# microsoft/fadtk

Measured on NVIDIA H100. Metric: audio_seconds_embedded_per_second, higher is better.
Workload: dtype f16

## Files before the change

fadtk_b200/csrc/conv_gemm.cuh:

```cuda
#pragma once
#include "sm90.cuh"

namespace fad {

struct ConvGemmParams {
    int taps;
    int cblks;
    int box_w, box_h, box_n;
    int tiles_w, tiles_h;
    int img_groups;
    int n_tiles;
    int H, W, NB, Cout;
    int lo_adds;
    int ld_out, n_valid;
    int relu, pool;
    const float* bias;
    __half* out;
    float* out_f32;
    float* resid;
    int resid_C, resid_res, resid_shift;
};

__device__ __forceinline__ long long window_row_to_token(long long o, int res, int shift) {
    const int lg_nw = 28 - __clz(res);
    const int nw = res >> 3;
    const int in = (int)(o & 63);
    const long long wi = o >> 6;
    const int wx = (int)wi & (nw - 1);
    const int wy = (int)(wi >> lg_nw) & (nw - 1);
    const long long b = wi >> (2 * lg_nw);
    int y = wy * 8 + (in >> 3) + shift, xx = wx * 8 + (in & 7) + shift;
    if (y >= res) y -= res;
    if (xx >= res) xx -= res;
    return (b * res + y) * res + xx;
}

constexpr int kTileM = 128;
constexpr int kBlockK = 64;
constexpr int kConvGemmThreads = 512;
constexpr int kConsumers = 2;
constexpr int kConsumerRegs = 168;
constexpr int kEpiRegs = 136;
constexpr int kClusterCtas = 2;
constexpr int kChunkSteps = 8;
constexpr float kAccumShrinkPerElement = 1.06e-9f;
constexpr uint32_t kABytes = kTileM * kBlockK * 2;
constexpr uint32_t kEpiRowBytes = 128 * 4;
constexpr uint32_t kEpiBytes = 64 * kEpiRowBytes;
constexpr uint32_t kBiasBytes = 128 * 4;
static_assert(40 + kEpiRegs + kConsumers * kConsumerRegs <= 65536 / 128, "register file over-subscribed");
static_assert(kConsumerRegs > 65536 / kConvGemmThreads, "the consumers raise their register count (setmaxnreg.inc)");

template <int N_TILE, int WMODE>
__host__ __device__ constexpr uint32_t conv_gemm_stage_bytes() {
    return kABytes + (WMODE == 1 ? 2 : 1) * N_TILE * kBlockK * 2;
}

template <int N_TILE, int STAGES, int WMODE>
__host__ __device__ constexpr uint32_t conv_gemm_smem_bytes() {
    return STAGES * conv_gemm_stage_bytes<N_TILE, WMODE>() + 1024  + 256
         + kConsumers * kEpiBytes + 4 * kBiasBytes;
}

__device__ __forceinline__ uint32_t pack_half2(float a, float b) {
    __half2 h = __floats2half2_rn(a, b);
    return *reinterpret_cast<uint32_t*>(&h);
}
template <int N>
__device__ __forceinline__ void gelu_erf_n(float* x) {
    float z[N], q[N];
#pragma unroll
    for (int i = 0; i < N; ++i) { z[i] = fminf(fabsf(x[i]) * 0.70710678118654752f, 4.3f); q[i] = 1.04899843e-04f; }
    constexpr float kQ[6] = {-4.92790774e-04f, -2.22368206e-03f, 2.93586859e-02f, -1.48908889e-01f, -9.18342944e-01f,
                             -1.62791250e+00f};
#pragma unroll
    for (int t = 0; t < 6; ++t) {
#pragma unroll
        for (int i = 0; i < N; ++i) q[i] = fmaf(q[i], z[i], kQ[t]);
    }
#pragma unroll
    for (int i = 0; i < N; ++i) asm("ex2.approx.ftz.f32 %0, %1;" : "=f"(q[i]) : "f"(q[i] * z[i]));
#pragma unroll
    for (int i = 0; i < N; ++i) x[i] = 0.5f * x[i] * (1.0f + copysignf(1.0f - q[i], x[i]));
}
__device__ __forceinline__ float gelu_erf(float x) {
    gelu_erf_n<1>(&x);
    return x;
}

template <int N>
__device__ __forceinline__ void elu_ex2_n(float* x) {
    float e[N], t[N];
#pragma unroll
    for (int i = 0; i < N; ++i) asm("ex2.approx.ftz.f32 %0, %1;" : "=f"(e[i]) : "f"(fminf(x[i], 0.f) * 1.4426950408889634f));
#pragma unroll
    for (int i = 0; i < N; ++i) t[i] = x[i] * fmaf(x[i], fmaf(x[i], fmaf(x[i], 4.16666667e-2f, 1.66666667e-1f), 0.5f), 1.0f);
#pragma unroll
    for (int i = 0; i < N; ++i) x[i] = x[i] > 0.f ? x[i] : (x[i] > -0.0625f ? t[i] : e[i] - 1.0f);
}

__device__ __forceinline__ uint32_t hmax2_u32(uint32_t a, uint32_t b) {
    __half2 r = __hmax2(*reinterpret_cast<__half2*>(&a), *reinterpret_cast<__half2*>(&b));
    return *reinterpret_cast<uint32_t*>(&r);
}

template <int N_TILE, int STAGES, int WMODE>
__global__ void __launch_bounds__(kConvGemmThreads, 1)
conv_gemm_kernel(const __grid_constant__ CUtensorMap map_x,
                 const __grid_constant__ CUtensorMap map_w,
                 const ConvGemmParams p)
{
    using namespace sm90;
    static_assert(N_TILE == 128, "one m64n128 accumulator per consumer warpgroup");
    static_assert(WMODE == 0 || WMODE == 1, "WMODE 0: fp16 weights, 1: fp16 hi/lo pair");
    static_assert(kClusterCtas == 2, "the work units below are M-tile pairs");
    constexpr bool SPLIT_W = WMODE == 1;
    constexpr uint32_t kStageBytes = conv_gemm_stage_bytes<N_TILE, WMODE>();
    constexpr int kBRows = (SPLIT_W ? 2 : 1) * N_TILE;
    constexpr int kGroups = N_TILE / 32;

    extern __shared__ uint8_t smem_raw[];
    uint8_t* smem = reinterpret_cast<uint8_t*>((reinterpret_cast<uintptr_t>(smem_raw) + 1023) & ~uintptr_t(1023));
    uint64_t* bars = reinterpret_cast<uint64_t*>(smem + STAGES * kStageBytes);
    uint64_t* full = bars;
    uint64_t* empty = bars + STAGES;
    uint64_t* epi_full = bars + 2 * STAGES;
    uint64_t* epi_empty = bars + 2 * STAGES + kConsumers;
    static_assert((2 * STAGES + 2 * kConsumers) * 8 <= 256, "barriers");
    uint8_t* epi = smem + STAGES * kStageBytes + 256;

    const int warp = threadIdx.x >> 5;
    const int lane = threadIdx.x & 31;
    const int ksteps = p.taps * p.cblks;
    const int n_chunks = (ksteps + kChunkSteps - 1) / kChunkSteps;
    const int chunk_len = (ksteps + n_chunks - 1) / n_chunks;
    const int m_tiles = p.img_groups * p.tiles_h * p.tiles_w;
    const int n_clusters = (int)gridDim.x / kClusterCtas;
    const int total_units = (m_tiles + 1) / 2 * p.n_tiles;

    if (warp == 0 && lane == 0) {
        tma_prefetch_desc(&map_x);
        tma_prefetch_desc(&map_w);
    }
    if (warp == 1 && lane == 0) {
        for (int s = 0; s < STAGES; ++s) { mbar_init(&full[s], 1); mbar_init(&empty[s], kClusterCtas * kConsumers * 4); }
        for (int c = 0; c < kConsumers; ++c) { mbar_init(&epi_full[c], 128); mbar_init(&epi_empty[c], 64); }
        mbar_fence_init();
    }
    cluster_sync();

    if (warp < 4) {
        setmaxnreg_dec<40>();
        if (warp == 0 && elect_one()) {
            const int rank = (int)cluster_ctarank();
            const int cluster = (int)cluster_index();
            constexpr int kHalfRows = kBRows / kClusterCtas;
            uint8_t* const w_half = smem + kABytes + rank * kHalfRows * 128;
            int s = 0; uint32_t ph = 0;
            for (int unit = cluster; unit < total_units; unit += n_clusters) {
                const int nt = unit % p.n_tiles;
                const int m = min(2 * (unit / p.n_tiles) + rank, m_tiles - 1);
                const int w0 = (m % p.tiles_w) * p.box_w;
                const int h0 = ((m / p.tiles_w) % p.tiles_h) * p.box_h;
                const int n0 = (m / (p.tiles_w * p.tiles_h)) * p.box_n;
                for (int ks = 0; ks < ksteps; ++ks) {
                    const int tap = ks / p.cblks;
                    const int cb = ks - tap * p.cblks;
                    int dh = 0, dw = 0;
                    if (p.taps == 9) { dh = tap / 3 - 1; dw = tap % 3 - 1; }
                    mbar_wait(&empty[s], ph ^ 1);
                    uint8_t* st = smem + s * kStageBytes;
                    mbar_expect_tx(&full[s], kStageBytes);
                    tma_load_4d(st, &map_x, &full[s], cb * kBlockK, w0 + dw, h0 + dh, n0);
                    tma_load_2d_multicast(w_half + s * kStageBytes, &map_w, &full[s], ks * kBlockK,
                                          nt * kBRows + rank * kHalfRows, (1u << kClusterCtas) - 1);
                    if (++s == STAGES) { s = 0; ph ^= 1; }
                }
            }
        }
    } else if (warp < 4 + 4 * kConsumers) {
        setmaxnreg_inc<kConsumerRegs>();
        const int cluster = (int)cluster_index();
        const int c = (warp >> 2) - 1;
        const int wq = warp & 3;
        const uint32_t epi_base = smem_u32(epi) + c * kEpiBytes;
        int s = 0; uint32_t ph = 0, eph = 0;
        auto release = [&](int st_) {
            __syncwarp();
            if (lane == 0) {
#pragma unroll
                for (int cta = 0; cta < kClusterCtas; ++cta) mbar_arrive_cluster(&empty[st_], cta);
            }
        };

        for (int unit = cluster; unit < total_units; unit += n_clusters) {
            float sum[64], acc[64];
#pragma unroll
            for (int i = 0; i < 64; ++i) sum[i] = 0.f;
            for (int ks0 = 0; ks0 < ksteps; ks0 += chunk_len) {
                const int ks1 = min(ks0 + chunk_len, ksteps);
                const float unshrink = kAccumShrinkPerElement * (float)((ks1 - ks0) * kBlockK * (SPLIT_W && p.lo_adds ? 2 : 1));
                int prev_s = -1;
                for (int ks = ks0; ks < ks1; ++ks) {
                    mbar_wait(&full[s], ph);
                    const uint32_t a_addr = smem_u32(smem + s * kStageBytes);
                    const uint64_t a_desc = kmajor_sw128_desc(a_addr + c * 64 * 128);
                    const uint64_t b_desc = kmajor_sw128_desc(a_addr + kABytes);
                    wgmma_fence();
#pragma unroll
                    for (int k = 0; k < kBlockK / 16; ++k) {
                        wgmma_m64n128k16_f16<0, 0>(acc, a_desc + 2 * k, b_desc + 2 * k, (ks > ks0) || (k > 0));
                        if (SPLIT_W)
                            wgmma_m64n128k16_f16<0, 0>(acc, a_desc + 2 * k, b_desc + 2 * k + (N_TILE * 128 / 16), 1);
                    }
                    wgmma_commit();
                    wgmma_wait<1>();
                    if (prev_s >= 0) release(prev_s);
                    prev_s = s;
                    if (++s == STAGES) { s = 0; ph ^= 1; }
                }
                wgmma_wait<0>();
                fence_regs(acc);
                release(prev_s);
#pragma unroll
                for (int i = 0; i < 64; ++i) sum[i] += fmaf(acc[i], unshrink, acc[i]);
            }

            mbar_wait(&epi_empty[c], eph ^ 1);
            const int fr = wq * 16 + (lane >> 2);
            const uint32_t x = ((lane & 3) >> 1) ^ (fr & 7);
            const uint32_t row_base = epi_base + fr * kEpiRowBytes + (lane & 1) * 8;
#pragma unroll
            for (int jl = 0; jl < 4; ++jl) {
                const uint32_t a = row_base + (((2 * jl) ^ x) << 4);
#pragma unroll
                for (int jh = 0; jh < 4; ++jh) {
#pragma unroll
                    for (int i = 0; i < 2; ++i) {
                        const int j = 4 * jh + jl;
                        sts64(a + i * 8 * kEpiRowBytes + jh * 128, sum[4 * j + 2 * i], sum[4 * j + 2 * i + 1]);
                    }
                }
            }
            mbar_arrive(&epi_full[c]);
            eph ^= 1;
        }
    } else {
        if constexpr (kEpiRegs > 65536 / kConvGemmThreads) setmaxnreg_inc<kEpiRegs>();
        else setmaxnreg_dec<kEpiRegs>();
        const int rank = (int)cluster_ctarank();
        const int cluster = (int)cluster_index();
        const int e = warp - 4 - 4 * kConsumers;
        const int c = e >> 1;
        const int rr = (e & 1) * 32 + lane;
        const int r = c * 64 + rr;
        const int bw = p.box_w, bh = p.box_h;
        const int pw = r % bw;
        const int phh = (r / bw) % bh;
        const int pn = r / (bw * bh);
        const uint32_t wrows = smem_u32(epi) + c * kEpiBytes + (e & 1) * 32 * kEpiRowBytes;
        const uint32_t row_mine = wrows + lane * kEpiRowBytes;
        const uint32_t bias_s = smem_u32(epi) + kConsumers * kEpiBytes + e * kBiasBytes;
        const int sw = lane & 7;
        const int cq = lane & 7, rq = lane >> 3;
        uint32_t eph = 0;
        const bool plain = p.tiles_w == 1 && p.tiles_h == 1 && bw == 1 && bh == 1;
        const bool f32_path = p.out_f32 != nullptr || p.resid != nullptr;
        auto prefetch_resid = [&](int nt_, int m_) {
            if (p.resid == nullptr || !plain) return;
            const int n_ = m_ * kTileM + r;
            if (n_ >= p.NB) return;
            const long long tok = p.resid_res ? window_row_to_token((long long)n_, p.resid_res, p.resid_shift) : (long long)n_;
            for (int cc = nt_ * N_TILE; cc < nt_ * N_TILE + N_TILE && cc < p.resid_C; cc += 32)
                asm volatile("prefetch.global.L2 [%0];" :: "l"(p.resid + tok * p.resid_C + cc));
        };
        if (cluster < total_units) prefetch_resid(cluster % p.n_tiles, 2 * (cluster / p.n_tiles) + rank);

        for (int unit = cluster; unit < total_units; unit += n_clusters) {
            const int nt = unit % p.n_tiles;
            const int m = 2 * (unit / p.n_tiles) + rank;
            if (unit + n_clusters < total_units)
                prefetch_resid((unit + n_clusters) % p.n_tiles, 2 * ((unit + n_clusters) / p.n_tiles) + rank);
            __syncwarp();
            {
                const float4 b = __ldg(reinterpret_cast<const float4*>(p.bias + nt * N_TILE) + lane);
                sts128(bias_s + lane * 16, __float_as_uint(b.x), __float_as_uint(b.y), __float_as_uint(b.z), __float_as_uint(b.w));
            }
            __syncwarp();

            int w, h, n;
            if (plain) { w = 0; h = 0; n = m * kTileM + r; }
            else {
                w = (m % p.tiles_w) * bw + pw;
                h = ((m / p.tiles_w) % p.tiles_h) * bh + phh;
                n = (m / (p.tiles_w * p.tiles_h)) * p.box_n + pn;
            }
            const bool valid = n < p.NB;
            const int ch0 = nt * N_TILE;
            long long out_off = -1, res_off = -1;
            if (valid && !p.pool) {
                out_off = (long long)((size_t(n) * p.H + h) * p.W + w) * p.ld_out;
                if (p.resid != nullptr)
                    res_off = (p.resid_res ? window_row_to_token((long long)n, p.resid_res, p.resid_shift) : (long long)n)
                              * p.resid_C;
            }

            mbar_wait(&epi_full[c], eph);
#pragma unroll 1
            for (int g = 0; g < kGroups; ++g) {
                float f[32];
#pragma unroll
                for (int j = 0; j < 8; ++j) {
                    const uint4 u = lds128(row_mine + g * 128 + ((j ^ sw) << 4));
                    const uint4 b = lds128(bias_s + g * 128 + j * 16);
                    f[4 * j + 0] = __uint_as_float(u.x) + __uint_as_float(b.x);
                    f[4 * j + 1] = __uint_as_float(u.y) + __uint_as_float(b.y);
                    f[4 * j + 2] = __uint_as_float(u.z) + __uint_as_float(b.z);
                    f[4 * j + 3] = __uint_as_float(u.w) + __uint_as_float(b.w);
                }
                if (p.relu == 1) {
#pragma unroll
                    for (int j = 0; j < 32; ++j) f[j] = fmaxf(f[j], 0.0f);
                } else if (p.relu == 2) {
#pragma unroll
                    for (int j = 0; j < 32; j += 8) gelu_erf_n<8>(f + j);
                } else if (p.relu == 3) {
#pragma unroll
                    for (int j = 0; j < 32; j += 8) elu_ex2_n<8>(f + j);
                }

                if (!p.pool) {
                    if (f32_path) {
                        if (p.out != nullptr && out_off >= 0) {
                            uint4* dst = reinterpret_cast<uint4*>(p.out + out_off + ch0 + g * 32);
#pragma unroll
                            for (int j = 0; j < 4; ++j)
                                if (ch0 + g * 32 + 8 * j < p.n_valid)
                                    dst[j] = make_uint4(pack_half2(f[8 * j], f[8 * j + 1]), pack_half2(f[8 * j + 2], f[8 * j + 3]),
                                                        pack_half2(f[8 * j + 4], f[8 * j + 5]), pack_half2(f[8 * j + 6], f[8 * j + 7]));
                        }
#pragma unroll
                        for (int j = 0; j < 8; ++j)
                            sts128(row_mine + g * 128 + ((j ^ sw) << 4), __float_as_uint(f[4 * j]), __float_as_uint(f[4 * j + 1]),
                                   __float_as_uint(f[4 * j + 2]), __float_as_uint(f[4 * j + 3]));
                        __syncwarp();
                        const int col = ch0 + g * 32 + cq * 4;
#pragma unroll
                        for (int hf = 0; hf < 2; ++hf) {
                            float4 v[4];
#pragma unroll
                            for (int it = 0; it < 4; ++it) {
                                const int x = (hf * 4 + it) * 4 + rq;
                                const uint4 u = lds128(wrows + x * kEpiRowBytes + g * 128 + ((cq ^ (x & 7)) << 4));
                                v[it] = make_float4(__uint_as_float(u.x), __uint_as_float(u.y), __uint_as_float(u.z), __uint_as_float(u.w));
                            }
                            if (p.out_f32 != nullptr) {
#pragma unroll
                                for (int it = 0; it < 4; ++it) {
                                    const long long off = __shfl_sync(0xffffffffu, out_off, (hf * 4 + it) * 4 + rq);
                                    if (off >= 0 && col < p.n_valid) *reinterpret_cast<float4*>(p.out_f32 + off + col) = v[it];
                                }
                            }
                            if (p.resid != nullptr && ch0 + g * 32 < p.resid_C) {
                                long long offs[4];
                                float4 xv[4];
#pragma unroll
                                for (int it = 0; it < 4; ++it) {
                                    offs[it] = __shfl_sync(0xffffffffu, res_off, (hf * 4 + it) * 4 + rq);
                                    if (offs[it] >= 0) xv[it] = *reinterpret_cast<const float4*>(p.resid + offs[it] + col);
                                }
#pragma unroll
                                for (int it = 0; it < 4; ++it) {
                                    if (offs[it] >= 0) {
                                        const float4 a = v[it];
                                        xv[it].x += a.x; xv[it].y += a.y; xv[it].z += a.z; xv[it].w += a.w;
                                        *reinterpret_cast<float4*>(p.resid + offs[it] + col) = xv[it];
                                    }
                                }
                            }
                        }
                    } else if (p.out != nullptr) {
                        const int seg = (g & ~1) * 128;
#pragma unroll
                        for (int j = 0; j < 4; ++j)
                            sts128(row_mine + seg + ((((g & 1) * 4 + j) ^ sw) << 4),
                                   pack_half2(f[8 * j], f[8 * j + 1]), pack_half2(f[8 * j + 2], f[8 * j + 3]),
                                   pack_half2(f[8 * j + 4], f[8 * j + 5]), pack_half2(f[8 * j + 6], f[8 * j + 7]));
                        if (g & 1) {
                            __syncwarp();
                            const int col = ch0 + (g - 1) * 32 + cq * 8;
#pragma unroll
                            for (int it = 0; it < 8; ++it) {
                                const int x = it * 4 + rq;
                                const uint4 v = lds128(wrows + x * kEpiRowBytes + seg + ((cq ^ (x & 7)) << 4));
                                const long long off = __shfl_sync(0xffffffffu, out_off, x);
                                if (off >= 0 && col < p.n_valid) *reinterpret_cast<uint4*>(p.out + off + col) = v;
                            }
                        }
                    }
                } else {
                    uint32_t h2[16];
#pragma unroll
                    for (int j = 0; j < 16; ++j) h2[j] = pack_half2(f[2 * j], f[2 * j + 1]);
#pragma unroll
                    for (int j = 0; j < 16; ++j) {
                        uint32_t o = __shfl_xor_sync(0xffffffffu, h2[j], 1);
                        h2[j] = hmax2_u32(h2[j], o);
                        o = __shfl_xor_sync(0xffffffffu, h2[j], bw);
                        h2[j] = hmax2_u32(h2[j], o);
                    }
                    const int sub = (pw & 1) | ((phh & 1) << 1);
                    uint4 o;
                    o.x = sub == 0 ? h2[0] : sub == 1 ? h2[4] : sub == 2 ? h2[8]  : h2[12];
                    o.y = sub == 0 ? h2[1] : sub == 1 ? h2[5] : sub == 2 ? h2[9]  : h2[13];
                    o.z = sub == 0 ? h2[2] : sub == 1 ? h2[6] : sub == 2 ? h2[10] : h2[14];
                    o.w = sub == 0 ? h2[3] : sub == 1 ? h2[7] : sub == 2 ? h2[11] : h2[15];
                    if (valid) {
                        const size_t pix = (size_t(n) * (p.H >> 1) + (h >> 1)) * (p.W >> 1) + (w >> 1);
                        *reinterpret_cast<uint4*>(p.out + pix * p.Cout + ch0 + g * 32 + sub * 8) = o;
                    }
                }
            }
            mbar_arrive(&epi_empty[c]);
            eph ^= 1;
        }
    }
    cluster_sync();
}

}
```

fadtk_b200/csrc/fadtk_b200.cu:

```cuda
#include "../../include/fadtk_b200.h"

#include <cuda.h>
#include <cuda_runtime.h>
#include <cuda_fp16.h>
#include <cxxabi.h>
#include <algorithm>
#include <cmath>
#include <cstdio>
#include <cstdlib>
#include <cstring>
#include <memory>
#include <set>
#include <string>
#include <type_traits>
#include <utility>
#include <vector>

#include "conv_gemm.cuh"
#include "frontend.cuh"
#include "stats.cuh"
#include "frechet.cuh"
#include "clap.cuh"
#include "resample.cuh"
#include "whisper.cuh"
#include "encodec.cuh"
#include "wav2vec.cuh"
#include "attention_wgmma.cuh"
#include "kad.cuh"
#include "prdc.cuh"

namespace {

thread_local std::string g_err;

int fail(const std::string& m) { g_err = m; return 1; }

#define CK(call)                                                                          \
    do {                                                                                  \
        cudaError_t e_ = (call);                                                          \
        if (e_ != cudaSuccess)                                                            \
            return fail(std::string(#call) + ": " + cudaGetErrorString(e_));              \
    } while (0)

class DeviceBuffer {
public:
    DeviceBuffer() = default;
    DeviceBuffer(DeviceBuffer&& o) noexcept : p_(o.p_), bytes_(o.bytes_) { o.p_ = nullptr; o.bytes_ = 0; }
    ~DeviceBuffer() { if (p_) cudaFree(p_); }

    int grow(size_t bytes) {
        if (bytes_ >= bytes) return 0;
        if (p_) cudaFree(p_);
        p_ = nullptr; bytes_ = 0;
        CK(cudaMalloc(&p_, bytes));
        bytes_ = bytes;
        return 0;
    }
    template <typename T = void> T* get() const { return static_cast<T*>(p_); }
    size_t size() const { return bytes_; }

private:
    void* p_ = nullptr;
    size_t bytes_ = 0;
};

template <typename T>
int upload(std::vector<DeviceBuffer>& mem, T** dst, const void* src, size_t bytes) {
    DeviceBuffer b;
    if (b.grow(bytes)) return 1;
    CK(cudaMemcpy(b.get(), src, bytes, cudaMemcpyHostToDevice));
    *dst = b.get<T>();
    mem.push_back(std::move(b));
    return 0;
}
template <typename T>
int alloc(std::vector<DeviceBuffer>& mem, T** dst, size_t bytes, bool zero = false) {
    DeviceBuffer b;
    if (b.grow(bytes)) return 1;
    if (zero) CK(cudaMemset(b.get(), 0, bytes));
    *dst = b.get<T>();
    mem.push_back(std::move(b));
    return 0;
}

int check_tensors(const char* fn, const void* const* t, int n_tensors) {
    for (int i = 0; i < n_tensors; ++i)
        if (!t[i]) return fail(std::string(fn) + ": null tensor pointer");
    return 0;
}

typedef CUresult (*EncodeTiledFn)(CUtensorMap*, CUtensorMapDataType, cuuint32_t, void*,
                                  const cuuint64_t*, const cuuint64_t*, const cuuint32_t*,
                                  const cuuint32_t*, CUtensorMapInterleave, CUtensorMapSwizzle,
                                  CUtensorMapL2promotion, CUtensorMapFloatOOBfill);

EncodeTiledFn get_encode_fn() {
    static EncodeTiledFn fn = nullptr;
    if (!fn) {
        void* p = nullptr;
        cudaDriverEntryPointQueryResult q;
        if (cudaGetDriverEntryPoint("cuTensorMapEncodeTiled", &p, cudaEnableDefault, &q) == cudaSuccess &&
            q == cudaDriverEntryPointSuccess)
            fn = reinterpret_cast<EncodeTiledFn>(p);
    }
    return fn;
}

int encode_f16_map(CUtensorMap* map, const void* base, int rank, const uint64_t* dims,
                   const uint64_t* strides_bytes , const uint32_t* box) {
    EncodeTiledFn fn = get_encode_fn();
    if (!fn) return fail("cuTensorMapEncodeTiled entry point not available");
    cuuint64_t gdim[5], gstr[4];
    cuuint32_t bdim[5], estr[5];
    for (int i = 0; i < rank; ++i) { gdim[i] = dims[i]; bdim[i] = box[i]; estr[i] = 1; }
    for (int i = 0; i + 1 < rank; ++i) gstr[i] = strides_bytes[i];
    CUresult r = fn(map, CU_TENSOR_MAP_DATA_TYPE_FLOAT16, (cuuint32_t)rank, const_cast<void*>(base),
                    gdim, gstr, bdim, estr, CU_TENSOR_MAP_INTERLEAVE_NONE, CU_TENSOR_MAP_SWIZZLE_128B,
                    CU_TENSOR_MAP_L2_PROMOTION_L2_256B, CU_TENSOR_MAP_FLOAT_OOB_FILL_NONE);
    if (r != CUDA_SUCCESS) {
        char buf[256];
        snprintf(buf, sizeof buf, "cuTensorMapEncodeTiled failed (%d) rank=%d dims=%llu,%llu box=%u,%u", (int)r, rank,
                 (unsigned long long)dims[0], (unsigned long long)(rank > 1 ? dims[1] : 0), box[0], rank > 1 ? box[1] : 0);
        return fail(buf);
    }
    return 0;
}

struct LayerGeom {
    int taps, Cin, Cout, H, W, relu, pool;
    int box_w, box_h, box_n, n_tile;
    int split_w;
};

int make_geom(LayerGeom& g, int H, int W, int Cin, int Cout, int taps, int relu, int pool, int split_w) {
    g.taps = taps; g.Cin = Cin; g.Cout = Cout; g.H = H; g.W = W; g.relu = relu; g.pool = pool;
    g.split_w = split_w;
    if (Cin % 64 != 0) return fail("Cin must be a multiple of 64");
    if (taps != 1 && taps != 9) return fail("taps must be 1 or 9");
    if (H == 1 && W == 1) { g.box_w = 1; g.box_h = 1; g.box_n = 128; }
    else {
        g.box_w = W < 16 ? W : 16;
        if (g.box_w != 8 && g.box_w != 16) return fail("W must be 8 or a multiple of 16");
        if (W % g.box_w != 0) return fail("W must be a multiple of the 16-pixel box");
        int bh = 1;
        while (bh * 2 <= 128 / g.box_w && H % (bh * 2) == 0) bh *= 2;
        g.box_h = bh;
        g.box_n = 128 / (g.box_w * g.box_h);
    }
    if (pool && (g.box_h % 2 != 0 || g.box_w % 2 != 0)) return fail("pooling needs even tile boxes");
    if (Cout % 128 != 0) return fail("Cout must be a multiple of 128");
    g.n_tile = 128;
    return 0;
}

struct VggState;
struct ClapState;
struct WhisperState;
struct EncodecState;
struct W2vState;

}

struct fad_handle {
    int device = 0;
    int num_sms = 0;
    int max_examples = 0;
    long long launches = 0;
    int gemm_clusters[2] = {};

    std::vector<DeviceBuffer> mem;
    double *d_twiddle = nullptr, *d_hann = nullptr, *d_melw = nullptr;
    int *d_mel_start = nullptr, *d_mel_count = nullptr;

    DeviceBuffer ws_tiles, ws_sums, gather_buf;
    DeviceBuffer fr_buf;
    DeviceBuffer rs_bank, rs_mono;
    int rs_in = 0, rs_out = 0;
    DeviceBuffer kad_buf;
    DeviceBuffer kad_agree;
    std::set<const void*> zero_lo;

    void* nccl_comm = nullptr;

    std::unique_ptr<VggState> vgg;
    std::unique_ptr<ClapState> clap;
    std::unique_ptr<WhisperState> whisper;
    std::unique_ptr<EncodecState> encodec;
    std::unique_ptr<W2vState> w2v;
    ~fad_handle();

    bool prof_on = false;
    std::vector<cudaEvent_t> ev_pool;
    size_t ev_used = 0;
    struct Span { int cat; size_t e0, e1; };
    std::vector<Span> spans;
    double prof_ms[FAD_PROF_CATEGORIES] = {};
    long long prof_count[FAD_PROF_CATEGORIES] = {};
};

namespace {

std::string kernel_name(const void* kernel) {
    const char* mangled = nullptr;
    if (cudaFuncGetName(&mangled, kernel) != cudaSuccess || !mangled) return "kernel launch";
    int status = 0;
    char* demangled = abi::__cxa_demangle(mangled, nullptr, nullptr, &status);
    const std::string name = demangled ? demangled : mangled;
    free(demangled);
    return name;
}

template <typename... Params, typename... Args>
int launch_attrs(fad_handle* h, void (*kernel)(Params...), dim3 grid, dim3 block, size_t smem, cudaStream_t st,
                 cudaLaunchAttribute* attrs, unsigned n_attrs, Args&&... args) {
    if (grid.x == 0 || grid.y == 0 || grid.z == 0) return 0;
    cudaLaunchConfig_t cfg = {};
    cfg.gridDim = grid;
    cfg.blockDim = block;
    cfg.dynamicSmemBytes = smem;
    cfg.stream = st;
    cfg.attrs = attrs;
    cfg.numAttrs = n_attrs;
    cudaError_t e = cudaLaunchKernelEx(&cfg, kernel, std::forward<Args>(args)...);
    const cudaError_t last = cudaGetLastError();
    if (e == cudaSuccess) e = last;
    if (e != cudaSuccess) return fail(kernel_name((const void*)kernel) + ": " + cudaGetErrorString(e));
    h->launches++;
    return 0;
}
template <typename... Params, typename... Args>
int launch(fad_handle* h, void (*kernel)(Params...), dim3 grid, dim3 block, size_t smem, cudaStream_t st, Args&&... args) {
    return launch_attrs(h, kernel, grid, block, smem, st, nullptr, 0, std::forward<Args>(args)...);
}

template <int WMODE> struct Gemm {
    static constexpr int kStages = WMODE ? 3 : 4;
    static constexpr uint32_t kSmem = fad::conv_gemm_smem_bytes<128, kStages, WMODE>();
    static_assert(kSmem <= 227 * 1024, "over the per-CTA shared-memory limit");
    static constexpr auto kernel = fad::conv_gemm_kernel<128, kStages, WMODE>;
};

cudaLaunchAttribute cta_pair() {
    cudaLaunchAttribute attr = {};
    attr.id = cudaLaunchAttributeClusterDimension;
    attr.val.clusterDim.x = fad::kClusterCtas; attr.val.clusterDim.y = 1; attr.val.clusterDim.z = 1;
    return attr;
}

template <int WMODE>
int setup_gemm(fad_handle* h) {
    CK(cudaFuncSetAttribute(Gemm<WMODE>::kernel, cudaFuncAttributeMaxDynamicSharedMemorySize, (int)Gemm<WMODE>::kSmem));
    cudaLaunchAttribute attr = cta_pair();
    cudaLaunchConfig_t cfg = {};
    cfg.gridDim = dim3(fad::kClusterCtas * (unsigned)h->num_sms);
    cfg.blockDim = dim3(fad::kConvGemmThreads);
    cfg.dynamicSmemBytes = Gemm<WMODE>::kSmem;
    cfg.attrs = &attr;
    cfg.numAttrs = 1;
    CK(cudaOccupancyMaxActiveClusters(&h->gemm_clusters[WMODE], Gemm<WMODE>::kernel, &cfg));
    if (h->gemm_clusters[WMODE] <= 0) return fail("conv_gemm_kernel: no CTA pair fits on the device");
    return 0;
}

template <int WMODE>
int launch_conv_gemm(fad_handle* h, const CUtensorMap& mx, const CUtensorMap& mw, const fad::ConvGemmParams& p, cudaStream_t st) {
    const int units = (p.img_groups * p.tiles_h * p.tiles_w + 1) / 2 * p.n_tiles;
    cudaLaunchAttribute attr = cta_pair();
    return launch_attrs(h, Gemm<WMODE>::kernel, dim3(fad::kClusterCtas * (unsigned)std::min(units, h->gemm_clusters[WMODE])),
                        dim3(fad::kConvGemmThreads), Gemm<WMODE>::kSmem, st, &attr, 1, mx, mw, p);
}

int encode_layer_maps(const LayerGeom& g, const void* x, long long nb_dim, const void* w,
                      CUtensorMap* mx, CUtensorMap* mw, int a_cols = 0, long long a_row_stride = 0) {
    const uint64_t ac = a_cols > 0 ? (uint64_t)a_cols : (uint64_t)g.Cin;
    const uint64_t xd[4] = {ac, (uint64_t)g.W, (uint64_t)g.H, (uint64_t)nb_dim};
    uint64_t xs[3] = {ac * 2, (uint64_t)g.W * ac * 2, (uint64_t)g.H * g.W * ac * 2};
    if (a_row_stride > 0) xs[0] = xs[1] = xs[2] = (uint64_t)a_row_stride * 2;
    const uint32_t xb[4] = {64, (uint32_t)g.box_w, (uint32_t)g.box_h, (uint32_t)g.box_n};
    if (encode_f16_map(mx, x, 4, xd, xs, xb)) return 1;
    const uint64_t K = (uint64_t)g.taps * g.Cin;
    const uint64_t rows_mul = g.split_w ? 2 : 1;
    const uint64_t wd[2] = {K, (uint64_t)g.Cout * rows_mul};
    const uint64_t ws[1] = {K * 2};
    const uint32_t wb[2] = {64, (uint32_t)(g.n_tile * rows_mul / fad::kClusterCtas)};
    return encode_f16_map(mw, w, 2, wd, ws, wb);
}

int launch_attention_wgmma(fad_handle* h, const __half* qkv, long long n_clips, int S, int d, int heads, __half* out, cudaStream_t st) {
    if (heads * 64 != d) return fail("attention_wgmma: head dimension must be 64");
    CUtensorMap map;
    const uint64_t dims[3] = {(uint64_t)3 * d, (uint64_t)S, (uint64_t)n_clips};
    const uint64_t strides[2] = {(uint64_t)3 * d * 2, (uint64_t)S * 3 * d * 2};
    const uint32_t box[3] = {64, 128, 1};
    if (encode_f16_map(&map, qkv, 3, dims, strides, box)) return 1;
    fad::AttnParams p;
    p.S = S; p.d = d; p.heads = heads; p.out = out;
    return launch(h, fad::attention_wgmma_kernel, dim3((S + 127) / 128, heads, (unsigned)n_clips), fad::kAtThreads, fad::kAtSmem,
                  st, map, p);
}

int run_layer(fad_handle* h, const LayerGeom& g, const CUtensorMap& mx, const CUtensorMap& mw, const void* w,
              int NB, const float* bias, void* out, float* out_f32, cudaStream_t st,
              float* resid = nullptr, int resid_C = 0, int resid_res = 0, int resid_shift = 0, int n_valid = 0) {
    fad::ConvGemmParams p;
    p.taps = g.taps; p.cblks = g.Cin / 64;
    p.box_w = g.box_w; p.box_h = g.box_h; p.box_n = g.box_n;
    p.tiles_w = g.W / g.box_w; p.tiles_h = g.H / g.box_h;
    p.img_groups = (NB + g.box_n - 1) / g.box_n;
    p.n_tiles = g.Cout / g.n_tile;
    p.H = g.H; p.W = g.W; p.NB = NB; p.Cout = g.Cout;
    p.n_valid = n_valid > 0 ? n_valid : g.Cout;
    p.ld_out = p.n_valid;
    p.relu = g.relu; p.pool = g.pool;
    p.bias = bias; p.out = reinterpret_cast<__half*>(out); p.out_f32 = out_f32;
    p.resid = resid; p.resid_C = resid_C; p.resid_res = resid_res; p.resid_shift = resid_shift;
    p.lo_adds = g.split_w == 1 && h->zero_lo.count(w) == 0;
    if (g.split_w) return launch_conv_gemm<1>(h, mx, mw, p, st);
    return launch_conv_gemm<0>(h, mx, mw, p, st);
}

__global__ void wlo_absmax_kernel(const __half* __restrict__ w, long long n_tiles, long long K, unsigned int* __restrict__ out) {
    float m = 0.f;
    const long long total = n_tiles * 128 * K;
    for (long long e = blockIdx.x * (long long)blockDim.x + threadIdx.x; e < total; e += (long long)gridDim.x * blockDim.x) {
        const long long row = e / K, k = e - row * K;
        const long long t = row >> 7, j = row & 127;
        m = fmaxf(m, fabsf(__half2float(w[((t * 256 + 128 + j) * K) + k])));
    }
    for (int o = 16; o > 0; o >>= 1) m = fmaxf(m, __shfl_xor_sync(0xffffffffu, m, o));
    if ((threadIdx.x & 31) == 0) atomicMax(out, __float_as_uint(m));
}
int note_split_weights(fad_handle* h, const void* w, long long n_tiles, long long K, cudaStream_t st) {
    DeviceBuffer d_max;
    if (d_max.grow(4)) return 1;
    unsigned int mx = 0;
    const unsigned blocks = (unsigned)std::max<long long>(1, std::min<long long>((n_tiles * 128 * K + 255) / 256, (long long)h->num_sms * 16));
    CK(cudaMemsetAsync(d_max.get(), 0, 4, st));
    if (launch(h, wlo_absmax_kernel, blocks, 256, 0, st, reinterpret_cast<const __half*>(w), n_tiles, K, d_max.get<unsigned int>()))
        return 1;
    CK(cudaMemcpyAsync(&mx, d_max.get(), 4, cudaMemcpyDeviceToHost, st));
    CK(cudaStreamSynchronize(st));
    if (mx == 0) h->zero_lo.insert(w); else h->zero_lo.erase(w);
    return 0;
}

int upload_split(fad_handle* h, std::vector<DeviceBuffer>& mem, __half** dst, const void* src, size_t n, size_t k) {
    if (upload(mem, dst, src, 2 * n * k * 2)) return 1;
    return note_split_weights(h, *dst, (long long)(n / 128), (long long)k, 0);
}

struct VggLayer { int H, W, Cin, Cout, taps, relu, pool; };
const VggLayer kVgg[8] = {
    {48, 32, 64, 128, 9, 1, 1},
    {24, 16, 128, 256, 9, 1, 0},
    {24, 16, 256, 256, 9, 1, 1},
    {12, 8, 256, 512, 9, 1, 0},
    {12, 8, 512, 512, 9, 1, 1},
    {1, 1, 12288, 4096, 1, 1, 0},
    {1, 1, 4096, 4096, 1, 1, 0},
    {1, 1, 4096, 128, 1, 0, 0},
};
const size_t kActElems[8] = {48 * 32 * 64, 24 * 16 * 128, 24 * 16 * 256, 12 * 8 * 256,
                             12 * 8 * 512, 6 * 4 * 512, 4096, 4096};

struct VggState {
    std::vector<DeviceBuffer> mem;
    float *conv1_w = nullptr, *conv1_b = nullptr;
    __half* w[8] = {};
    float* b[8] = {};
    float* logmel = nullptr;
    __half* act[8] = {};
    CUtensorMap map_x[8], map_w[8];
    LayerGeom geom[8];
};

void build_frontend_tables(std::vector<double>& tw, std::vector<double>& hann,
                           std::vector<double>& melw, std::vector<int>& mstart, std::vector<int>& mcount) {
    const double PI = 3.14159265358979323846;
    tw.resize(512); hann.resize(fad::kWin);
    for (int k = 0; k < 256; ++k) {
        tw[2 * k] = std::cos(-2.0 * PI * k / 512.0);
        tw[2 * k + 1] = std::sin(-2.0 * PI * k / 512.0);
    }
    for (int n = 0; n < fad::kWin; ++n) hann[n] = 0.5 - 0.5 * std::cos(2.0 * PI / fad::kWin * n);
    auto mel = [](double f) { return 1127.0 * std::log(1.0 + f / 700.0); };
    std::vector<double> bins(fad::kBins), edges(fad::kMel + 2);
    for (int i = 0; i < fad::kBins; ++i) bins[i] = mel(8000.0 * i / (fad::kBins - 1));
    const double lo = mel(125.0), hi = mel(7500.0);
    for (int i = 0; i < fad::kMel + 2; ++i) edges[i] = lo + (hi - lo) * i / (fad::kMel + 1);
    melw.assign(fad::kMel * fad::kMelMaxTaps, 0.0);
    mstart.assign(fad::kMel, 0); mcount.assign(fad::kMel, 0);
    for (int b = 0; b < fad::kMel; ++b) {
        const double l = edges[b], c = edges[b + 1], u = edges[b + 2];
        int first = -1, cnt = 0;
        for (int i = 1; i < fad::kBins; ++i) {
            const double w = std::fmax(0.0, std::fmin((bins[i] - l) / (c - l), (u - bins[i]) / (u - c)));
            if (w > 0.0) {
                if (first < 0) first = i;
                const int off = i - first;
                if (off < fad::kMelMaxTaps) { melw[b * fad::kMelMaxTaps + off] = w; cnt = off + 1; }
            }
        }
        mstart[b] = first < 0 ? 0 : first;
        mcount[b] = cnt;
    }
}

size_t prof_begin(fad_handle* h, cudaStream_t st) {
    if (!h->prof_on) return 0;
    if (h->ev_used == h->ev_pool.size()) { cudaEvent_t e; cudaEventCreate(&e); h->ev_pool.push_back(e); }
    cudaEventRecord(h->ev_pool[h->ev_used], st);
    return h->ev_used++;
}
void prof_end(fad_handle* h, int cat, size_t e0, cudaStream_t st) {
    if (!h->prof_on) return;
    const size_t e1 = prof_begin(h, st);
    h->spans.push_back({cat, e0, e1});
}

template <typename In>
int launch_stats_dmma(fad_handle* h, const In* E, long long n_rows, int d, const __half* shift, double* acc, cudaStream_t st) {
    constexpr bool kProf = sizeof(In) == 2;
    if (d <= 0 || d % 64 != 0) return fail("d must be a positive multiple of 64");
    fad::StatsDmmaParams p;
    p.n_rows = n_rows; p.d = d; p.n_tiles = d / fad::kSdTile;
    p.n_pairs = p.n_tiles * (p.n_tiles + 1) / 2;
    const long long stages = (n_rows + fad::kSdRows - 1) / fad::kSdRows;
    long long want = (4LL * h->num_sms + p.n_pairs - 1) / p.n_pairs;
    if (want < 1) want = 1;
    long long per = (stages + want - 1) / want;
    if (per < 4) per = 4;
    p.n_splits = (int)((stages + per - 1) / per);
    p.rows_per_split = per * fad::kSdRows;
    p.shift = shift;
    const size_t jobs = (size_t)p.n_pairs * p.n_splits;
    if (h->ws_tiles.grow(jobs * fad::kSdTile * fad::kSdTile * 8)) return 1;
    if (h->ws_sums.grow((size_t)p.n_tiles * p.n_splits * fad::kSdTile * 8)) return 1;
    p.ws_tiles = h->ws_tiles.get<double>(); p.ws_sums = h->ws_sums.get<double>();
    size_t ev = kProf ? prof_begin(h, st) : 0;
    if (launch(h, fad::stats_dmma_kernel<In>, (unsigned)jobs, 256, 0, st, E, p)) return 1;
    if (kProf) { prof_end(h, FAD_PROF_STATS, ev, st); ev = prof_begin(h, st); }
    if (launch(h, fad::stats_dmma_reduce_kernel, dim3(p.n_pairs, fad::kSdTile * fad::kSdTile / 256), 256, 0, st, p, acc)) return 1;
    if (kProf) prof_end(h, FAD_PROF_STATS_REDUCE, ev, st);
    return 0;
}

}

extern "C" {

int fad_version(void) { return 1; }

int fad_profile_enable(fad_handle* h, int on) {
    if (!h) return fail("null handle");
    h->prof_on = on != 0;
    return 0;
}

int fad_profile_collect(fad_handle* h, double* ms_out, long long* count_out, int reset) {
    if (!h) return fail("null handle");
    CK(cudaSetDevice(h->device));
    CK(cudaDeviceSynchronize());
    for (const auto& sp : h->spans) {
        float ms = 0.f;
        if (cudaEventElapsedTime(&ms, h->ev_pool[sp.e0], h->ev_pool[sp.e1]) == cudaSuccess) {
            h->prof_ms[sp.cat] += ms; h->prof_count[sp.cat]++;
        }
    }
    h->spans.clear(); h->ev_used = 0;
    for (int i = 0; i < FAD_PROF_CATEGORIES; ++i) {
        if (ms_out) ms_out[i] = h->prof_ms[i];
        if (count_out) count_out[i] = h->prof_count[i];
        if (reset) { h->prof_ms[i] = 0.0; h->prof_count[i] = 0; }
    }
    return 0;
}
const char* fad_last_error(void) { return g_err.c_str(); }

int fad_create(int device, int max_examples, fad_handle** out) {
    if (!out) return fail("null out pointer");
    int count = 0;
    if (cudaGetDeviceCount(&count) != cudaSuccess || count == 0)
        return fail("no CUDA device: fadtk_b200 has no CPU fallback");
    if (device < 0 || device >= count) return fail("bad device index");
    CK(cudaSetDevice(device));
    cudaDeviceProp prop;
    CK(cudaGetDeviceProperties(&prop, device));
    if (prop.major != 9) return fail("fadtk_b200 kernels are built for sm_90a (Hopper H100) only");
    std::unique_ptr<fad_handle> h(new fad_handle());
    h->device = device;
    h->num_sms = prop.multiProcessorCount;
    h->max_examples = max_examples > 0 ? max_examples : 2048;

    std::vector<double> tw, hann, melw; std::vector<int> ms, mc;
    build_frontend_tables(tw, hann, melw, ms, mc);
    if (upload(h->mem, &h->d_twiddle, tw.data(), tw.size() * 8) || upload(h->mem, &h->d_hann, hann.data(), hann.size() * 8) ||
        upload(h->mem, &h->d_melw, melw.data(), melw.size() * 8) || upload(h->mem, &h->d_mel_start, ms.data(), ms.size() * 4) ||
        upload(h->mem, &h->d_mel_count, mc.data(), mc.size() * 4)) return 1;
    const auto smem = [](const void* kernel, size_t bytes) {
        return cudaFuncSetAttribute(kernel, cudaFuncAttributeMaxDynamicSharedMemorySize, (int)bytes);
    };
    CK(smem((const void*)fad::logmel_kernel<double>, fad::logmel_smem_bytes<double>()));
    CK(smem((const void*)fad::logmel_kernel<float>, fad::logmel_smem_bytes<float>()));
    CK(smem((const void*)fad::clap_logmel_kernel, fad::clap_logmel_smem_bytes()));
    CK(smem((const void*)fad::attention_wgmma_kernel, fad::kAtSmem));
    CK(smem((const void*)fad::clap_window_attention_kernel<24>, fad::att_smem_bytes(24, fad::kAttWarps, fad::kAttStages)));
    CK(smem((const void*)fad::clap_window_attention_kernel<32>, fad::att_smem_bytes(32, fad::kAttWarps, fad::kAttStages)));
    CK(smem((const void*)fad::kad_tile_kernel<0>, fad::kKadSmemBytes));
    CK(smem((const void*)fad::kad_tile_kernel<1>, fad::kKadSmemBytes));
    CK(smem((const void*)fad::kad_tile_kernel<2>, fad::kKadSmemBytes));
    CK(smem((const void*)fad::prdc_tile_kernel<0>, fad::kPrdcSmemBytes));
    CK(smem((const void*)fad::prdc_tile_kernel<1>, fad::kPrdcSmemBytes));
    if (setup_gemm<0>(h.get()) || setup_gemm<1>(h.get())) return 1;
    *out = h.release();
    return 0;
}

int fad_destroy(fad_handle* h) {
    if (!h) return 0;
    cudaSetDevice(h->device);
    fad_comm_destroy(h);
    delete h;
    return 0;
}

long long fad_launch_count(fad_handle* h) { return h ? h->launches : 0; }

int fad_vggish_load(fad_handle* h, const fad_vggish_weights* w) {
    if (!h || !w) return fail("null argument");
    const void* src[18] = {w->conv1_w_host, w->conv1_b_host,
                           w->conv_w_host[0], w->conv_w_host[1], w->conv_w_host[2], w->conv_w_host[3], w->conv_w_host[4],
                           w->fc_w_host[0], w->fc_w_host[1], w->fc_w_host[2],
                           w->conv_b_host[0], w->conv_b_host[1], w->conv_b_host[2], w->conv_b_host[3], w->conv_b_host[4],
                           w->fc_b_host[0], w->fc_b_host[1], w->fc_b_host[2]};
    if (check_tensors("fad_vggish_load", src, 18)) return 1;
    const void* const* wsrc = src + 2;
    const void* const* bsrc = src + 10;
    CK(cudaSetDevice(h->device));
    h->vgg.reset();
// ... 949 lines not shown
```

Measured before the change: 182,100.

## Halve epilogue staging buffer and overlap next tile's first chunk with hand-off

The epilogue staging buffer is cut to 64 columns per consumer, and the accumulator is handed to the epilogue warps in two halves. The consumer issues the first k-step of the next tile's GEMM between the two half hand-offs, so tensor-core work overlaps the register-to-shared drain. Bias staging is now shared per consumer pair behind named barriers. The freed shared memory buys one extra pipeline stage for both weight modes. The cost is more synchronisation round-trips and a more complex control flow.

```diff
diff --git a/fadtk_b200/csrc/conv_gemm.cuh b/fadtk_b200/csrc/conv_gemm.cuh
--- a/fadtk_b200/csrc/conv_gemm.cuh
+++ b/fadtk_b200/csrc/conv_gemm.cuh
@@ -1,4 +1,5 @@
 #pragma once
+#include <type_traits>
 #include "sm90.cuh"
 
 namespace fad {
@@ -45,7 +46,7 @@
 constexpr int kChunkSteps = 8;
 constexpr float kAccumShrinkPerElement = 1.06e-9f;
 constexpr uint32_t kABytes = kTileM * kBlockK * 2;
-constexpr uint32_t kEpiRowBytes = 128 * 4;
+constexpr uint32_t kEpiRowBytes = 64 * 4;
 constexpr uint32_t kEpiBytes = 64 * kEpiRowBytes;
 constexpr uint32_t kBiasBytes = 128 * 4;
 static_assert(40 + kEpiRegs + kConsumers * kConsumerRegs <= 65536 / 128, "register file over-subscribed");
@@ -59,7 +60,7 @@
 template <int N_TILE, int STAGES, int WMODE>
 __host__ __device__ constexpr uint32_t conv_gemm_smem_bytes() {
     return STAGES * conv_gemm_stage_bytes<N_TILE, WMODE>() + 1024  + 256
-         + kConsumers * kEpiBytes + 4 * kBiasBytes;
+         + kConsumers * (kEpiBytes + kBiasBytes);
 }
 
 __device__ __forceinline__ uint32_t pack_half2(float a, float b) {
@@ -193,39 +194,9 @@
             }
         };
 
-        for (int unit = cluster; unit < total_units; unit += n_clusters) {
-            float sum[64], acc[64];
-#pragma unroll
-            for (int i = 0; i < 64; ++i) sum[i] = 0.f;
-            for (int ks0 = 0; ks0 < ksteps; ks0 += chunk_len) {
-                const int ks1 = min(ks0 + chunk_len, ksteps);
-                const float unshrink = kAccumShrinkPerElement * (float)((ks1 - ks0) * kBlockK * (SPLIT_W && p.lo_adds ? 2 : 1));
-                int prev_s = -1;
-                for (int ks = ks0; ks < ks1; ++ks) {
-                    mbar_wait(&full[s], ph);
-                    const uint32_t a_addr = smem_u32(smem + s * kStageBytes);
-                    const uint64_t a_desc = kmajor_sw128_desc(a_addr + c * 64 * 128);
-                    const uint64_t b_desc = kmajor_sw128_desc(a_addr + kABytes);
-                    wgmma_fence();
-#pragma unroll
-                    for (int k = 0; k < kBlockK / 16; ++k) {
-                        wgmma_m64n128k16_f16<0, 0>(acc, a_desc + 2 * k, b_desc + 2 * k, (ks > ks0) || (k > 0));
-                        if (SPLIT_W)
-                            wgmma_m64n128k16_f16<0, 0>(acc, a_desc + 2 * k, b_desc + 2 * k + (N_TILE * 128 / 16), 1);
-                    }
-                    wgmma_commit();
-                    wgmma_wait<1>();
-                    if (prev_s >= 0) release(prev_s);
-                    prev_s = s;
-                    if (++s == STAGES) { s = 0; ph ^= 1; }
-                }
-                wgmma_wait<0>();
-                fence_regs(acc);
-                release(prev_s);
-#pragma unroll
-                for (int i = 0; i < 64; ++i) sum[i] += fmaf(acc[i], unshrink, acc[i]);
-            }
-
+        float sum[64], acc[64];
+        auto hand_off = [&](auto half) {
+            constexpr int h = decltype(half)::value;
             mbar_wait(&epi_empty[c], eph ^ 1);
             const int fr = wq * 16 + (lane >> 2);
             const uint32_t x = ((lane & 3) >> 1) ^ (fr & 7);
@@ -234,16 +205,70 @@
             for (int jl = 0; jl < 4; ++jl) {
                 const uint32_t a = row_base + (((2 * jl) ^ x) << 4);
 #pragma unroll
-                for (int jh = 0; jh < 4; ++jh) {
+                for (int jh = 0; jh < 2; ++jh) {
 #pragma unroll
                     for (int i = 0; i < 2; ++i) {
-                        const int j = 4 * jh + jl;
+                        const int j = 4 * (2 * h + jh) + jl;
                         sts64(a + i * 8 * kEpiRowBytes + jh * 128, sum[4 * j + 2 * i], sum[4 * j + 2 * i + 1]);
                     }
                 }
             }
             mbar_arrive(&epi_full[c]);
             eph ^= 1;
+        };
+
+        int prev_s = -1;
+        auto issue_chunk = [&](int ks0, int from, int to) -> float {
+            const int ks1 = min(ks0 + chunk_len, ksteps);
+            if (from == ks0) prev_s = -1;
+            for (int ks = from; ks < (to > 0 ? to : ks1); ++ks) {
+                mbar_wait(&full[s], ph);
+                const uint32_t a_addr = smem_u32(smem + s * kStageBytes);
+                const uint64_t a_desc = kmajor_sw128_desc(a_addr + c * 64 * 128);
+                const uint64_t b_desc = kmajor_sw128_desc(a_addr + kABytes);
+                wgmma_fence();
+#pragma unroll
+                for (int k = 0; k < kBlockK / 16; ++k) {
+                    wgmma_m64n128k16_f16<0, 0>(acc, a_desc + 2 * k, b_desc + 2 * k, (ks > ks0) || (k > 0));
+                    if (SPLIT_W)
+                        wgmma_m64n128k16_f16<0, 0>(acc, a_desc + 2 * k, b_desc + 2 * k + (N_TILE * 128 / 16), 1);
+                }
+                wgmma_commit();
+                wgmma_wait<1>();
+                if (prev_s >= 0) release(prev_s);
+                prev_s = s;
+                if (++s == STAGES) { s = 0; ph ^= 1; }
+            }
+            return kAccumShrinkPerElement * (float)((ks1 - ks0) * kBlockK * (SPLIT_W && p.lo_adds ? 2 : 1));
+        };
+        auto retire_chunk = [&]() {
+            wgmma_wait<0>();
+            fence_regs(acc);
+            release(prev_s);
+        };
+
+        if (cluster < total_units) {
+            float unshrink = issue_chunk(0, 0, 0);
+            for (int unit = cluster;; unit += n_clusters) {
+                retire_chunk();
+#pragma unroll
+                for (int i = 0; i < 64; ++i) sum[i] = 0.f + fmaf(acc[i], unshrink, acc[i]);
+                for (int ks0 = chunk_len; ks0 < ksteps; ks0 += chunk_len) {
+                    unshrink = issue_chunk(ks0, ks0, 0);
+                    retire_chunk();
+#pragma unroll
+                    for (int i = 0; i < 64; ++i) sum[i] += fmaf(acc[i], unshrink, acc[i]);
+                }
+                if (unit + n_clusters >= total_units) {
+                    hand_off(std::integral_constant<int, 0>());
+                    hand_off(std::integral_constant<int, 1>());
+                    break;
+                }
+                issue_chunk(0, 0, 1);
+                hand_off(std::integral_constant<int, 0>());
+                unshrink = issue_chunk(0, 1, 0);
+                hand_off(std::integral_constant<int, 1>());
+            }
         }
     } else {
         if constexpr (kEpiRegs > 65536 / kConvGemmThreads) setmaxnreg_inc<kEpiRegs>();
@@ -260,7 +285,7 @@
         const int pn = r / (bw * bh);
         const uint32_t wrows = smem_u32(epi) + c * kEpiBytes + (e & 1) * 32 * kEpiRowBytes;
         const uint32_t row_mine = wrows + lane * kEpiRowBytes;
-        const uint32_t bias_s = smem_u32(epi) + kConsumers * kEpiBytes + e * kBiasBytes;
+        const uint32_t bias_s = smem_u32(epi) + kConsumers * kEpiBytes + c * kBiasBytes;
         const int sw = lane & 7;
         const int cq = lane & 7, rq = lane >> 3;
         uint32_t eph = 0;
@@ -281,12 +306,12 @@
             const int m = 2 * (unit / p.n_tiles) + rank;
             if (unit + n_clusters < total_units)
                 prefetch_resid((unit + n_clusters) % p.n_tiles, 2 * ((unit + n_clusters) / p.n_tiles) + rank);
-            __syncwarp();
-            {
+            named_bar_sync(1 + c, 64);
+            if ((e & 1) == 0) {
                 const float4 b = __ldg(reinterpret_cast<const float4*>(p.bias + nt * N_TILE) + lane);
                 sts128(bias_s + lane * 16, __float_as_uint(b.x), __float_as_uint(b.y), __float_as_uint(b.z), __float_as_uint(b.w));
             }
-            __syncwarp();
+            named_bar_sync(1 + c, 64);
 
             int w, h, n;
             if (plain) { w = 0; h = 0; n = m * kTileM + r; }
@@ -305,13 +330,14 @@
                               * p.resid_C;
             }
 
-            mbar_wait(&epi_full[c], eph);
 #pragma unroll 1
             for (int g = 0; g < kGroups; ++g) {
+                const uint32_t gs = (g & 1) * 128;
+                if (gs == 0) mbar_wait(&epi_full[c], eph);
                 float f[32];
 #pragma unroll
                 for (int j = 0; j < 8; ++j) {
-                    const uint4 u = lds128(row_mine + g * 128 + ((j ^ sw) << 4));
+                    const uint4 u = lds128(row_mine + gs + ((j ^ sw) << 4));
                     const uint4 b = lds128(bias_s + g * 128 + j * 16);
                     f[4 * j + 0] = __uint_as_float(u.x) + __uint_as_float(b.x);
                     f[4 * j + 1] = __uint_as_float(u.y) + __uint_as_float(b.y);
@@ -341,7 +367,7 @@
                         }
 #pragma unroll
                         for (int j = 0; j < 8; ++j)
-                            sts128(row_mine + g * 128 + ((j ^ sw) << 4), __float_as_uint(f[4 * j]), __float_as_uint(f[4 * j + 1]),
+                            sts128(row_mine + gs + ((j ^ sw) << 4), __float_as_uint(f[4 * j]), __float_as_uint(f[4 * j + 1]),
                                    __float_as_uint(f[4 * j + 2]), __float_as_uint(f[4 * j + 3]));
                         __syncwarp();
                         const int col = ch0 + g * 32 + cq * 4;
@@ -351,7 +377,7 @@
 #pragma unroll
                             for (int it = 0; it < 4; ++it) {
                                 const int x = (hf * 4 + it) * 4 + rq;
-                                const uint4 u = lds128(wrows + x * kEpiRowBytes + g * 128 + ((cq ^ (x & 7)) << 4));
+                                const uint4 u = lds128(wrows + x * kEpiRowBytes + gs + ((cq ^ (x & 7)) << 4));
                                 v[it] = make_float4(__uint_as_float(u.x), __uint_as_float(u.y), __uint_as_float(u.z), __uint_as_float(u.w));
                             }
                             if (p.out_f32 != nullptr) {
@@ -380,10 +406,9 @@
                             }
                         }
                     } else if (p.out != nullptr) {
-                        const int seg = (g & ~1) * 128;
 #pragma unroll
                         for (int j = 0; j < 4; ++j)
-                            sts128(row_mine + seg + ((((g & 1) * 4 + j) ^ sw) << 4),
+                            sts128(row_mine + ((((g & 1) * 4 + j) ^ sw) << 4),
                                    pack_half2(f[8 * j], f[8 * j + 1]), pack_half2(f[8 * j + 2], f[8 * j + 3]),
                                    pack_half2(f[8 * j + 4], f[8 * j + 5]), pack_half2(f[8 * j + 6], f[8 * j + 7]));
                         if (g & 1) {
@@ -392,7 +417,7 @@
 #pragma unroll
                             for (int it = 0; it < 8; ++it) {
                                 const int x = it * 4 + rq;
-                                const uint4 v = lds128(wrows + x * kEpiRowBytes + seg + ((cq ^ (x & 7)) << 4));
+                                const uint4 v = lds128(wrows + x * kEpiRowBytes + ((cq ^ (x & 7)) << 4));
                                 const long long off = __shfl_sync(0xffffffffu, out_off, x);
                                 if (off >= 0 && col < p.n_valid) *reinterpret_cast<uint4*>(p.out + off + col) = v;
                             }
@@ -420,9 +445,11 @@
                         *reinterpret_cast<uint4*>(p.out + pix * p.Cout + ch0 + g * 32 + sub * 8) = o;
                     }
                 }
-            }
-            mbar_arrive(&epi_empty[c]);
-            eph ^= 1;
+                if (gs != 0) {
+                    mbar_arrive(&epi_empty[c]);
+                    eph ^= 1;
+                }
+            }
         }
     }
     cluster_sync();
diff --git a/fadtk_b200/csrc/fadtk_b200.cu b/fadtk_b200/csrc/fadtk_b200.cu
--- a/fadtk_b200/csrc/fadtk_b200.cu
+++ b/fadtk_b200/csrc/fadtk_b200.cu
@@ -234,7 +234,7 @@
 }
 
 template <int WMODE> struct Gemm {
-    static constexpr int kStages = WMODE ? 3 : 4;
+    static constexpr int kStages = WMODE ? 4 : 5;
     static constexpr uint32_t kSmem = fad::conv_gemm_smem_bytes<128, kStages, WMODE>();
     static_assert(kSmem <= 227 * 1024, "over the per-CTA shared-memory limit");
     static constexpr auto kernel = fad::conv_gemm_kernel<128, kStages, WMODE>;
```

Measured after the change: 188,800, median of 6. 3.7% higher.
